# SahakyanLab/GenomeAssembler_dev

Measured on AMD Instinct MI355X. Metric: k-mers built+scored/sec, higher is better.
Workload: dtype u64 keys / u32 counts / f64 scores; 1 GPU; cfg2 (configs[2]): 100 x 50000 bp segments per GPU, 150 bp reads at 50x, k=31, build + breakage scoring of all contigs; mode=segments, segments_total=100, distinct_kmers_rank0=3843627, parallelism=segments sharded over 1 GPU(s), no collective

## Files before the change

### genomeassembler_dev_amd/csrc/kernels.h

```cpp
#pragma once
#include <hip/hip_runtime.h>
#include <stdint.h>

#include "device_utils.h"
#include "keyops.h"

struct ReadSet {
    const u64* words;
    const u64* read_off;
    const u64* seg_read_off;
    const u32* seg_tile_start;
    const uint4* tile_info;
    u32 fixed_len;
    u32 n_segments;
};

__device__ __forceinline__ void read_span(const ReadSet& rs, u64 r, u64* p0, u32* len) {
    if (rs.fixed_len) { *p0 = rs.read_off ? rs.read_off[r] : r * rs.fixed_len; *len = rs.fixed_len; }
    else { const u64 a = rs.read_off[r]; *p0 = a; *len = (u32)(rs.read_off[r + 1] - a); }
}

struct GraphView {
    const void* dk_key;
    const u32* dstart;
// ... 60 lines not shown
    GASM_OVF_TIP_RANK = 4,
};
static_assert(GASM_FLAG_ACTIVE + GASM_FLAG_ACTIVE_N <= GASM_FLAG_WORDS && GASM_FLAG_WORDS * 4 == GASM_FLAG_BYTES, "flag area layout");

template <class W>
struct BuildReport {
    W* w;
    u32 S;
    __host__ __device__ W& dstart(u32 s) const { return w[s]; }
    __host__ __device__ W& cstart(u32 s) const { return (w + S + 1)[s]; }
    __host__ __device__ W& bstart_lo(u32 s) const { return (w + 2 * S + 2)[2 * s]; }
    __host__ __device__ W& bstart_hi(u32 s) const { return (w + 2 * S + 2)[2 * s + 1]; }
    __host__ __device__ W& flags() const { return w[4 * S + 4]; }
    __host__ __device__ W& rank_failed() const { return w[4 * S + 5]; }
    __host__ __device__ W& ticket() const { return w[4 * S + 6]; }
    static size_t words(u32 S) { return 4 * (size_t)S + 8; }
};

__global__ void k_pack_ascii(const u8* ascii, u64 nbases_host, const u64* nbases_dev, u64* words, u32* err);
#define GASM_TILE_WG 512
template <class K> __global__ void k_tile_hist(ReadSet rs, const uint4* tinfo, int k, int bbits, u32 g, u32 n_tiles, ushort4* tcnt);
__global__ void k_tile_scan(ReadSet rs, int bbits, u32 padm, const ushort4* tcnt, u32* toff, u32* hist, u32* flags);
template <class TO> __global__ void k_scan_excl(const u32* in, TO* out, u32 n);
__global__ void k_copy_u64(const u64* a, u64* b, u32 n);
template <class K>
__global__ void k_bucket_scatter(ReadSet rs, const uint4* tinfo, int k, int bbits, u32 g, u32 padm, u32 n_tiles, const u64* bstart, const u32* toff,
                                 const ushort4* tcnt, K* keys, u64 scratch);
#define GASM_RT_MAX 16
template <class K>
__global__ void k_bucket_partition(ReadSet rs, const uint4* tinfo, int k, int bbits, u32 g, u32 padm, u32 n_tiles, const u64* bstart, u32* cursor,
                                   K* keys, u64 scratch, u32* flags);
template <class K, int TBL>
__global__ void k_bucket_dedup(K* keys, u32* mult, const u64* bstart, const u32* blen, u32* bucket_d, u32* overflow, u16* fdir, int low_bits, int dbg,
                               unsigned long long* stamps, u32* dstart);
#define GASM_BUCKET_MAX 65535
template <class K>
__global__ void k_bucket_dedup_multi(const K* keys, K* keys_out, u32* mult, const u64* bstart, u32* bucket_d, u32* overflow, u16* fdir, int low_bits);
template <class K>
__global__ void k_bucket_solid(K* keys, u32* mult, const u64* bstart, u32* bucket_d, u16* fdir, int low_bits, int fbits, int bbits, u32 min_count,
                               u32* removed, u32* done, u32* dstart);
template <class K>
__global__ void k_tip_mark(GraphView gv, u32 n_segments, u32 chunks, const u8* eflag, const u32* clen, const u32* nxt, const u32* dk_cnt, const u64* bstart,
                           u32* mult, u32 tip_len, u32* flags, u32* tips);
template <class K>
__global__ void k_bubble_mark(GraphView gv, u32 n_segments, u32 chunks, const u8* eflag, const u32* clen, const u32* nxt, const u32* dk_cnt, const u64* bstart,
                              u32* mult, u32 bubble_len, u32* flags, u32* bubbles);
__global__ void k_kmer_spectrum(const u32* dstart, u32 nb, const u32* dk_cnt, u32 n_segments, u32 chunks, u32* hist);
template <class K>
__global__ void k_lowcov_mark(GraphView gv, u32 n_segments, u32 chunks, const u8* eflag, const u32* clen, const u32* nxt, const u32* dk_cnt, const u64* bstart,
                              u32* mult, u32 cov_len, u32 cov_cutoff, u32* flags, u32* removed);
__global__ void k_contig_cov(const u32* dstart, u32 nb, u32 n_segments, u32 chunks, const u64* link, const u32* e_cid, const u32* dk_cnt,
                             const u32* seg_cstart, unsigned long long* msum, u32* nedges);
template <class K>
__global__ void k_bucket_gather(const K* keys, const u32* mult, const u64* bstart, const u32* dstart, K* dk_key, u32* dk_cnt, u32* claim, u8* eflag,
                                u32* flags);
template <class K> __global__ void k_edge_target(GraphView gv, u32 n_segments, u32 chunks, u32* tgt, u32* claim);
__global__ void k_edge_multi(GraphView gv, u32 n_segments, u32 chunks, const u32* tgt, const u32* claim, u8* eflag);
template <class K>
__global__ void k_node_flags(GraphView gv, u32 n_segments, u32 chunks, const u32* claim, u8* eflag, u64* link, u32* clen);
__global__ void k_edge_next(GraphView gv, u32 n_segments, u32 chunks, const u32* tgt, const u8* eflag, u32* nxt, u64* link);
__global__ void k_link_jump(GraphView gv, u32 n_segments, u32 chunks, u64* link, const u32* prev_active, u32* active, int jumps, const u32* nxt,
                            u32* clen);
__global__ void k_rank_rulers(GraphView gv, u32 n_segments, u32 chunks, u64* link, u32* rtab, u32 rshift, u32* flags);
__global__ void k_rank_lds(GraphView gv, const u32* rtab, u64* link, int max_rounds, u32 rshift, u32 lds_entries, u32* flags);
__global__ void k_chain_len(const u32* nxt, const u64* link, u32* clen, const u32* n_edges_p);
__global__ void k_contig_scan(GraphView gv, const u8* eflag, const u32* clen, u32* e_cid, u64* e_coff, u32* seg_ncontig,
                              u64* seg_cbases, u32* done, u32* seg_cstart, u64* seg_bstart, const u32* flags, u32* report, u32 ticket);
__global__ void k_contig_place(GraphView gv, const u8* eflag, const u32* seg_cstart, const u64* seg_bstart, u32* e_cid, u64* e_coff,
                               u64* c_off, u32 n_segments, u32 chunks);
template <class K>
__global__ void k_contig_emit(GraphView gv, const u64* link, const u32* nxt, const u64* e_coff, u8* out, u32 n_segments, u32 chunks);
__global__ void k_reads_both_strands(const u64* words, const u64* read_off, const u64* seg_read_off, u32 fixed_len, u32 n_segments, u64 n_reads, u32 g,
                                     unsigned long long* out);
template <class K>
__global__ void k_contig_twin(GraphView gv, const u64* link, const u32* e_cid, const u64* c_off, const u32* seg_cstart, const u8* text, u32 n_segments,
                              u32* twin, u32* bad);

template <class K>
__global__ void k_pack_runs(const K* keys, const u32* mult, const u64* bstart, const u32* bucket_d, const u32* gb_list, const u64* dst_off, K* out_keys,
                            u32* out_cnt);
template <class K, int TBL>
__global__ void k_bucket_merge(const K* in_keys, const u32* in_cnt, const u64* run_off, const u32* run_len, u32 n_src, K* out_keys, u32* out_cnt,
                               const u64* bstart, u32* bucket_d, u32* overflow, u16* fdir, int low_bits, const u64* src_base);
__global__ void k_repack_reads(const u64* src, const u64* dir, u64* words_out);
__global__ void k_piece_positions(const u64* piece_first, const u64* piece_word_off, u32 n_pieces, u64 n_reads, u32 fixed_len, u64* pos);
__global__ void k_slice_last(const u32* a, const u64* off, u32 n, u32* out);

__global__ void k_chain_expand(const u64* cwords, const u64* c_off, const u64* sig_off, const u32* elem_contig, const u32* elem_skip, const u64* elem_pos,
                               const u64* out_off, u32 n_scaffolds, u64* out, u64 n_words);
struct ChainSigs {
    const u64* sig_off;
    const u32* elem_contig;
    const u32* elem_skip;
    const u64* elem_pos;
};
__global__ void k_str_bitonic(const u64* words, const u64* off, u32* idx, u32 n_pow2, u32 kk, u32 j, ChainSigs cs);
__global__ void k_str_bitonic_block(const u64* words, const u64* off, u32* idx, u32 n_pow2, u32 kk, u32 j0, ChainSigs cs);
__global__ void k_str_adjacent_eq(const u64* words, const u64* off, const u32* idx, u32 n, u8* same_as_prev, ChainSigs cs);
__global__ void k_unpack_ascii(const u64* words, u64 nbases, u8* out);
__global__ void k_guided_chain(PathSet ps, const unsigned long long* fx, int k, u32* g_next, u32* g_prev, u32* dbg_order);
__global__ void k_asm_match(const u64* cwords, const u64* c_off, u32 n, int k, u8* match, u8* row_any, u8* level_any);
__global__ void k_asm_merge(const u32* perm, u32 rows, u32 n, int k, const u32* clen, const u8* match, const u8* row_any, const u8* level_any,
                            const u64* cwords, const u64* c_off, u32* out_next, u8* out_ov, u32* out_heads, u32* out_nchains, u8* need_host);

__global__ void k_sim_weights(const u64* gwords, const u64* gbase, const u64* woff, u32 n_segments, int kmer, const long long* fixw, u64* w);
template <class T> __global__ void k_seg_scan_incl(T* a, const u64* off);
__global__ void k_sim_draw(const u64* cum, const u64* woff, const u64* doff, const u64* glen, u64 seed, u32 read_len, u32* start, u32* keep);
__global__ void k_sim_compact(const u32* start, const u32* keep, const u32* rank, const u64* doff, const u64* seg_read_off, u32* kept_start);
__global__ void k_sim_extract(const u64* gwords, const u64* gbase, const u64* seg_read_off, const u32* kept_start, u32 read_len, unsigned long long* out);

template <int LS>
__global__ void k_read_kmer_count(const u64* words, const u64* read_off, const u64* seg_read_off, u32 fixed_len, u32 n_segments, u32* out);

#define GASM_CORRECT_STATS 6
#define GASM_CORRECT_KMER_CAP 4096
template <class K>
__global__ void k_read_correct(ReadSet rs, GraphView gv, int have_graph, u32 reads_per_wg, u32 chunks, unsigned long long* out_words, u32* stats);

#define GASM_THREAD_KMER_CAP 4096
template <class K>
__global__ void k_contig_links(GraphView gv, const u64* link, const u32* e_cid, const u64* c_off, const u32* seg_cstart, const u8* text, u32 n_segments, u32* succ,
                               u32* pred);
template <class K>
__global__ void k_read_thread(ReadSet rs, GraphView gv, const u64* link, const u32* e_cid, const u64* c_off, const u32* seg_cstart, const u8* text, int have_graph, u32 span_len,
                              u32 reads_per_wg, u32 chunks, u32* link_support, u32* span_support, unsigned long long* skipped);
#define GASM_PAIR_COUNTERS 6
template <class K>
__global__ void k_pair_place(ReadSet rs, GraphView gv, const u64* link, const u32* e_cid, const u64* c_off, const u32* seg_cstart, int have_graph, u32 orient, u32 max_insert,
                             u64 n_pairs, u32 chunks, int32_t* rec, u32* hist, unsigned long long* counters);

struct SeedTable {
    u64* seed;
    u32* gpos;
    const u64* tbl_off;
};
__global__ void k_read_insert(ReadSet rs, SeedTable st, int w);
__global__ void k_path_scan(ReadSet rs, PathSet ps, SeedTable st, const u64* seg_base_off, int w, const u64* first_off, u32* first, u32 seg0,
                            u32 path_lo, u32 path_hi);
__global__ void k_first_to_poscnt(const u32* first, u64 n, u32* poscnt);
#define GASM_SCORE_MAX_TABLES 8
struct FixTables { const long long* p[GASM_SCORE_MAX_TABLES]; };
struct ProbTables { const double* p[GASM_SCORE_MAX_TABLES]; };
template <class K, int T>
__global__ void k_score_reads_graph(ReadSet rs, GraphView gv, const u64* link, const u32* e_cid, PathSet ps, FixTables dfix, int kmer,
                                    u32 reads_per_wg, u32 chunks, u32 lds_paths, u32* cnt, unsigned long long* sum, u64 sum_stride, int verify,
                                    u32* verify_flag);
__global__ void k_levenshtein(PathSet ps, u32 n_paths, const u64* twords, u32 nt, int infix, u8* carry_ws, u64 carry_stride, int32_t* out);
__global__ void k_levenshtein2(PathSet ps, u32 n_paths, const u64* twords, u32 nt, int infix, uint4* carry_ws, u64 carry_stride, int32_t* out);
__global__ void k_score_zero(u32* cnt, unsigned long long* sum, u64 sum_stride, u32 n_tables, const u32* n_paths_p);
__global__ void k_score_finish(PathSet ps, const u32* cnt, const unsigned long long* sum, const long long* dfix, const u64* seg_empty,
                               int kmer, double inv_scale, double* bp_score, double* norm_freq, double* norm_len, int32_t* kmer_breaks,
                               int32_t* seq_len, const u32* n_paths_p);
template <int T>
__global__ void k_path_reduce(PathSet ps, const u32* poscnt, const u32* extra, ProbTables dprob, int kmer, double* bp_score, double* norm_freq,
                              double* norm_len, u64 out_stride, int32_t* kmer_breaks, int32_t* seq_len, u32 n_paths);
__global__ void k_path_freq(PathSet ps, const u32* poscnt, const u32* total, const int32_t* drow, int kmer, u32 n_table,
                            u32* freq_cnt, u32 n_paths);
__global__ void k_ks_genome_hist(const u64* gwords, u64 glen, int kmer, const int32_t* drow, u32* hist);
__global__ void k_path_ks(PathSet ps, const u32* poscnt, const int32_t* drow, int kmer, u32 n_table, const double* pv, const u32* cumy, u32* scratch,
                          double* out, u32 n_paths, const u32* list);
__global__ void k_path_ks2(PathSet ps, const u32* poscnt, const int32_t* drow, int kmer, u32 n_table, const double* pv, const u32* cumy, const u32* run_end,
                           u32* scratch, double* out, u32* flags, u32 n_paths, u32 bins);
__global__ void k_cover_mark(const long long* start, const long long* len, u64 n, long long seq_len, int* diff);
__global__ void k_cover_count(const int* diff, long long seq_len, unsigned long long* covered);
__global__ void k_prob_dist(PathSet ps, const double* dprob, int kmer, const u64* pd_off, double* out, u32 n_paths);

template <class T>
struct XReport {
    T* w;
    u32 W;
    __host__ __device__ T& send_tot(u32 d) const { return w[d]; }
    __host__ __device__ T& recv_tot(u32 d) const { return w[W + d]; }
    __host__ __device__ T& info(u32 j) const { return w[2 * W + j]; }
    __host__ __device__ T& flags() const { return w[2 * W + 4]; }
    __host__ __device__ T& ticket() const { return w[2 * W + 5]; }
    static size_t words(u32 W) { return 2 * (size_t)W + 6; }
};
__global__ void k_x_flag_word(const u32* flags, u32* row_tail);
__global__ void k_x1_plan(const u32* lens_all, u64 stride, u32 nbt, const u32* order, const u32* dst_first, const u32* mine, u32 n_mine, u32 W, u32 r, u32 limit,
                          u64* send_off, u64* send_tot, u64* run_off, u32* run_len, u64* recv_tot, u64* bstart, u32* flags_or);
__global__ void k_x2_fill(u32* G, u32 nbt, const u32* mine, u32 n_mine, const u32* bucket_d, const u32* flags);
__global__ void k_x2_plan(const u32* G, const u16* own1, u32 W, u32 r, u32 gb_lo, u32 n_out, int bbits, const u32* mine, u32 n_mine, const u32* seg_first,
                          u64* send_off, u64* send_tot, u64* run_off, u32* run_len, u64* recv_tot, u64* bstart, u64* info);
__global__ void k_x_report(const u64* send_tot, const u64* recv_tot, u32 W, const u64* info, u32 n_info, const u32* flags_or, u64* report, u64 ticket);
__global__ void k_x_add_u32(u32* acc, const u32* v, u64 n);
```

### genomeassembler_dev_amd/csrc/kernels_build.hip

```cpp
#include "device_utils.h"
#include "keyops.h"
#include "kernels.h"
#include "dedup_order.h"

typedef unsigned long long u64x2 __attribute__((ext_vector_type(2)));

typedef unsigned int u32x4nt __attribute__((ext_vector_type(4)));
#ifndef GASM_NO_NT
__device__ __forceinline__ uint4 stream_load16(const uint4* p) {
    const u32x4nt v = __builtin_nontemporal_load(reinterpret_cast<const u32x4nt*>(p));
    return make_uint4(v.x, v.y, v.z, v.w);
}
#define GASM_STREAM_LOAD(p) stream_load16(p)
#define GASM_STREAM_STORE(v, p) __builtin_nontemporal_store((v), (p))
#else
#define GASM_STREAM_LOAD(p) (*(p))
#define GASM_STREAM_STORE(v, p) (*(p) = (v))
#endif

__global__ void __launch_bounds__(GASM_WG) k_pack_ascii(const u8* __restrict__ ascii, u64 nbases_host, const u64* __restrict__ nbases_dev,
                                                        u64* __restrict__ words, u32* __restrict__ err) {
    const u64 nbases = nbases_dev ? *nbases_dev : nbases_host;
    const u64 nwords = (nbases + 31) / 32 + 4;
    bool ok = true;
// ... 800 lines not shown
                keys[beg + pos] = rk[q];
                mult[beg + pos] = rc[q];
                atomicAdd(&s_bin[kfield(rk[q], bshift) & (bins - 1)], 1u);
                ++pos;
            }
        }
        out += tot;
        __syncthreads();
    }
    __syncthreads();
    {
        const u32 per = bins / GASM_WG;
        u32 c[4], sum = 0;
#pragma unroll
        for (u32 q = 0; q < 4; ++q) { c[q] = q < per ? s_bin[threadIdx.x * per + q] : 0u; sum += c[q]; }
        u32 tot;
        u32 ex = block_excl_scan<GASM_WG>(sum, s_tmp, &tot);
        u16* const row = fdir + (u64)bucket * (bins + 1);
#pragma unroll
        for (u32 q = 0; q < 4; ++q)
            if (q < per) { row[threadIdx.x * per + q] = (u16)ex; ex += c[q]; }
        if (threadIdx.x == GASM_WG - 1) row[bins] = (u16)ex;
    }
    if (threadIdx.x == 0) {
        publish_u32(&bucket_d[bucket], out);
        if (d > out) atomicAdd(&removed[bucket >> bbits], d - out);
    }
    dedup_last_scan(bucket_d, dstart, gridDim.x, done, s_tmp + 7, s_tmp);
}
template __global__ void k_bucket_solid<u64>(u64*, u32*, const u64*, u32*, u16*, int, int, int, u32, u32*, u32*, u32*);
template __global__ void k_bucket_solid<K128>(K128*, u32*, const u64*, u32*, u16*, int, int, int, u32, u32*, u32*, u32*);

__global__ void __launch_bounds__(GASM_WG) k_kmer_spectrum(const u32* __restrict__ dstart, u32 nb, const u32* __restrict__ dk_cnt, u32 n_segments,
                                                           u32 chunks, u32* __restrict__ hist) {
    __shared__ u32 s_h[256];
    s_h[threadIdx.x] = 0;
    __syncthreads();
    u32 seg, chunk;
    if (!seg_chunk(n_segments, chunks, &seg, &chunk)) return;
    for_seg_edges(dstart, nb, n_segments, chunks, [&](u32, u32, u32, u32 i) {
        const u32 m = dk_cnt[i];
        atomicAdd(&s_h[m < 255u ? m : 255u], 1u);
    });
    __syncthreads();
    const u32 v = s_h[threadIdx.x];
    if (v) atomicAdd(&hist[(u64)seg * 256 + threadIdx.x], v);
}
static_assert(GASM_WG == 256, "k_kmer_spectrum: one thread per bin");

template <class K>
__global__ void __launch_bounds__(GASM_WG) k_bucket_gather(const K* __restrict__ keys, const u32* __restrict__ mult,
                                                           const u64* __restrict__ bstart, const u32* __restrict__ dstart,
                                                           K* __restrict__ dk_key, u32* __restrict__ dk_cnt, u32* __restrict__ claim,
                                                           u8* __restrict__ eflag, u32* __restrict__ flags) {
    const u32 bucket = blockIdx.x;
    if (bucket == 0 && threadIdx.x != GASM_FLAG_OVERFLOW && threadIdx.x < GASM_FLAG_WORDS) flags[threadIdx.x] = 0;
    const u64 src = bstart[bucket];
    const u32 dst = dstart[bucket], d = dstart[bucket + 1] - dst;
    for (u32 i = threadIdx.x; i < d; i += GASM_WG) {
        dk_key[dst + i] = keys[src + i];
        dk_cnt[dst + i] = mult[src + i];
        claim[dst + i] = GASM_NONE32;
        eflag[dst + i] = 0;
    }
}
template __global__ void k_bucket_gather<u64>(const u64*, const u32*, const u64*, const u32*, u64*, u32*, u32*, u8*, u32*);
template __global__ void k_bucket_gather<K128>(const K128*, const u32*, const u64*, const u32*, K128*, u32*, u32*, u8*, u32*);

template <class K>
__device__ __forceinline__ bool kmer_exists(const GraphView& gv, u32 seg, const K& t) {
    u32 hi;
    const u32 j = graph_lower_bound<K>(gv, seg, t, &hi);
    return j < hi && keq(reinterpret_cast<const K*>(gv.dk_key)[j], t);
}

template <class K>
__global__ void __launch_bounds__(GASM_WG) k_edge_target(GraphView gv, u32 n_segments, u32 chunks, u32* __restrict__ tgt,
                                                         u32* __restrict__ claim) {
    const K* dk = reinterpret_cast<const K*>(gv.dk_key);
    for_seg_edges(gv.dstart, 1u << gv.bbits, n_segments, chunks, [&](u32 seg, u32, u32, u32 i) {
        const K v = klowbits(dk[i], 2 * (gv.k - 1));
        u32 bhi;
        const u32 j = graph_lower_bound<K>(gv, seg, kshl(v, 2), &bhi);
        const bool valid = j < bhi && keq(kshr(dk[j], 2), v);
        tgt[i] = valid ? j : GASM_NONE32;
        if (valid) claim[j] = i;
    });
}
template __global__ void k_edge_target<u64>(GraphView, u32, u32, u32*, u32*);
template __global__ void k_edge_target<K128>(GraphView, u32, u32, u32*, u32*);

__global__ void __launch_bounds__(GASM_WG) k_edge_multi(GraphView gv, u32 n_segments, u32 chunks, const u32* __restrict__ tgt,
                                                        const u32* __restrict__ claim, u8* __restrict__ eflag) {
    for_seg_edge_groups(gv.dstart, 1u << gv.bbits, n_segments, chunks, [&](u32, u32, u32, const u32 (&i)[GASM_EDGE_ILP], const bool (&ok)[GASM_EDGE_ILP]) {
        u32 j[GASM_EDGE_ILP], c[GASM_EDGE_ILP];
#pragma unroll
        for (int q = 0; q < GASM_EDGE_ILP; ++q) j[q] = ok[q] ? tgt[i[q]] : GASM_NONE32;
#pragma unroll
        for (int q = 0; q < GASM_EDGE_ILP; ++q) c[q] = j[q] != GASM_NONE32 ? claim[j[q]] : 0u;
#pragma unroll
        for (int q = 0; q < GASM_EDGE_ILP; ++q)
            if (j[q] != GASM_NONE32 && c[q] != i[q]) eflag[j[q]] = 2;
    });
}

template <class K>
__global__ void __launch_bounds__(GASM_WG) k_node_flags(GraphView gv, u32 n_segments, u32 chunks, const u32* __restrict__ claim,
                                                        u8* __restrict__ eflag, u64* __restrict__ link, u32* __restrict__ clen) {
    const K* dk = reinterpret_cast<const K*>(gv.dk_key);
    for_seg_edges(gv.dstart, 1u << gv.bbits, n_segments, chunks, [&](u32, u32 lo, u32 hi, u32 i) {
        const K u = kshr(dk[i], 2);
        u32 r = i;
        while (r > lo && keq(kshr(dk[r - 1], 2), u)) --r;
        u32 e = i + 1;
        while (e < hi && keq(kshr(dk[e], 2), u)) ++e;
        const u32 outd = e - r;
        const bool in_one = claim[r] != GASM_NONE32 && !(eflag[r] & 2);
        eflag[i] = (eflag[i] & 2) | ((!in_one || outd != 1) ? 1 : 0);
        clen[i] = 0;
    });
}
template __global__ void k_node_flags<u64>(GraphView, u32, u32, const u32*, u8*, u64*, u32*);
template __global__ void k_node_flags<K128>(GraphView, u32, u32, const u32*, u8*, u64*, u32*);

__global__ void __launch_bounds__(GASM_WG) k_edge_next(GraphView gv, u32 n_segments, u32 chunks, const u32* __restrict__ tgt,
                                                       const u8* __restrict__ eflag, u32* __restrict__ nxt, u64* __restrict__ link) {
    for_seg_edge_groups(gv.dstart, 1u << gv.bbits, n_segments, chunks, [&](u32, u32, u32, const u32 (&i)[GASM_EDGE_ILP], const bool (&ok)[GASM_EDGE_ILP]) {
        u32 j[GASM_EDGE_ILP], efi[GASM_EDGE_ILP], efj[GASM_EDGE_ILP];
#pragma unroll
        for (int q = 0; q < GASM_EDGE_ILP; ++q) { j[q] = ok[q] ? tgt[i[q]] : GASM_NONE32; efi[q] = ok[q] ? (u32)eflag[i[q]] : 0u; }
#pragma unroll
        for (int q = 0; q < GASM_EDGE_ILP; ++q) efj[q] = j[q] != GASM_NONE32 ? (u32)eflag[j[q]] : 1u;
#pragma unroll
        for (int q = 0; q < GASM_EDGE_ILP; ++q) {
            if (!ok[q]) continue;
            const u32 n = (j[q] != GASM_NONE32 && !(efj[q] & 1)) ? j[q] : GASM_NONE32;
            nxt[i[q]] = n;
            const u64 me_head = (efi[q] & 1) ? GASM_LINK_DONE : 0ull;
            if (n != GASM_NONE32) link[n] = ((u64)i[q] << 32) | me_head | 1ull;
            if (me_head) link[i[q]] = ((u64)i[q] << 32) | GASM_LINK_DONE;
        }
    });
}

#define GASM_JUMP_ILP 4
__global__ void __launch_bounds__(GASM_WG) k_link_jump(GraphView gv, u32 n_segments, u32 chunks, u64* __restrict__ link,
                                                       const u32* __restrict__ prev_active, u32* __restrict__ active, int jumps,
                                                       const u32* __restrict__ nxt, u32* __restrict__ clen) {
    if (prev_active && *prev_active == 0) return;
    u32 seg, chunk;
    if (!seg_chunk(n_segments, chunks, &seg, &chunk)) return;
    const u32 nb = 1u << gv.bbits;
    const u32 lo = gv.dstart[seg * nb], hi = gv.dstart[(seg + 1) * nb];
    for (u32 base = chunk * (GASM_WG * GASM_JUMP_ILP); base < hi - lo; base += chunks * (GASM_WG * GASM_JUMP_ILP)) {
        const u32 i0 = lo + base + threadIdx.x;
        u64 l[GASM_JUMP_ILP];
        bool act[GASM_JUMP_ILP];
#pragma unroll
        for (int q = 0; q < GASM_JUMP_ILP; ++q) {
            const u32 i = i0 + q * GASM_WG;
            l[q] = i < hi ? link[i] : ~0ull;
            act[q] = (u32)(l[q] >> 32) != GASM_NONE32 && !(l[q] & GASM_LINK_DONE);
        }
        const bool mine = act[0] || act[1] || act[2] || act[3];
        u32 tail = 0;
        if (nxt) {
#pragma unroll
            for (int q = 0; q < GASM_JUMP_ILP; ++q) {
                const u32 i = i0 + q * GASM_WG;
                if (i < hi && (act[q] || !prev_active) && nxt[i] == GASM_NONE32) tail |= 1u << q;
            }
        }
        for (int j = 0; j < jumps && (act[0] || act[1] || act[2] || act[3]); ++j) {
            u64 la[GASM_JUMP_ILP];
#pragma unroll
            for (int q = 0; q < GASM_JUMP_ILP; ++q)
                la[q] = act[q] ? __hip_atomic_load(&link[(u32)(l[q] >> 32)], __ATOMIC_RELAXED, __HIP_MEMORY_SCOPE_WORKGROUP) : 0ull;
#pragma unroll
            for (int q = 0; q < GASM_JUMP_ILP; ++q) {
                if (!act[q]) continue;
                if ((u32)(la[q] >> 32) == GASM_NONE32) { l[q] = ~0ull; act[q] = false; continue; }
                if (l[q] & GASM_LINK_TAG) {
                    if (!(la[q] & GASM_LINK_DONE)) { l[q] = ~0ull; act[q] = false; continue; }
                    l[q] = (la[q] & (0xFFFFFFFF00000000ull | GASM_LINK_DONE)) | (u64)((((u32)la[q] & 0x7FFFFFFFu) - ((u32)l[q] & 0x3FFFFFFFu)) & 0x3FFFFFFFu);
                    act[q] = false;
                    continue;
                }
                l[q] = (la[q] & (0xFFFFFFFF00000000ull | GASM_LINK_DONE)) | (u64)(((u32)l[q] + (u32)la[q]) & 0x7FFFFFFFu);
                if (l[q] & GASM_LINK_DONE) act[q] = false;
            }
        }
#pragma unroll
        for (int q = 0; q < GASM_JUMP_ILP; ++q)
// ... 518 lines not shown
```

### genomeassembler_dev_amd/csrc/kernels_score.hip

```cpp
#include "device_utils.h"
#include "kernels.h"

#define GASM_DIRECT_ROWS 87380
__device__ __forceinline__ u32 direct_base(u32 L) { return ((1u << (2 * L)) - 4u) / 3u; }

__device__ __forceinline__ bool break_window(const u64* __restrict__ words, u64 pbase, u32 plen, u32 j, int kmer, u32* idx) {
    const int st = (int)j - kmer / 2;
    const u32 start = st > 0 ? (u32)st : 0u;
    u32 width = 8;
    if (start == 0) {
        if (j == 1) width = 2;
        else if (j == 2) width = 4;
        else if (j == 3) width = 6;
    }
    if (start >= plen) return false;
    const u32 avail = plen - start;
    const u32 wd = width < avail ? width : avail;
    *idx = direct_base(wd) + (u32)kmer_at(words, pbase + start, (int)wd);
    return true;
}

__global__ void __launch_bounds__(GASM_WG) k_read_insert(ReadSet rs, SeedTable st, int w) {
    const u32 seg = blockIdx.y;
    const u64 r = rs.seg_read_off[seg] + (u64)blockIdx.x * GASM_WG + threadIdx.x;
// ... 131 lines not shown
        s_cnt[i] = 0;
    }
    __syncthreads();
    for (u64 r = r0 + threadIdx.x; r < r1; r += GASM_WG) {
        u32 c = 0;
        u64 pb = 0, pe = 0;
        const u64 g = graph_match<K>(rs, gv, link, e_cid, ps, seg, r, &c, &pb, &pe, verify, verify_flag);
        if (g == ~0ull) continue;
        const u32 plen = (u32)(pe - pb);
        u32 idx = 0;
        const bool hit = break_window(ps.words, pb, plen, (u32)(g - pb), kmer, &idx);
        long long fx[T];
#pragma unroll
        for (int t = 0; t < T; ++t) fx[t] = hit ? dfix.p[t][idx] : 0;
        if (in_lds) {
            atomicAdd(&s_cnt[c - pfirst], 1u);
#pragma unroll
            for (int t = 0; t < T; ++t) atomicAdd(&s_sum[(size_t)t * lds_paths + (c - pfirst)], (unsigned long long)fx[t]);
        } else {
            atomicAdd(&cnt[c], 1u);
#pragma unroll
            for (int t = 0; t < T; ++t) atomicAdd(&sum[(u64)t * sum_stride + c], (unsigned long long)fx[t]);
        }
    }
    __syncthreads();
    if (in_lds) for (u32 i = threadIdx.x; i < np; i += GASM_WG) {
        const u32 c = s_cnt[i];
        if (c) {
            atomicAdd(&cnt[pfirst + i], c);
#pragma unroll
            for (int t = 0; t < T; ++t) atomicAdd(&sum[(u64)t * sum_stride + pfirst + i], s_sum[(size_t)t * lds_paths + i]);
        }
    }
}

#define GASM_INST_SCORE(K, T)                                                                                                         \
    template __global__ void k_score_reads_graph<K, T>(ReadSet, GraphView, const u64*, const u32*, PathSet, FixTables, int, u32, u32, u32, u32*, \
                                                       unsigned long long*, u64, int, u32*);
#define GASM_INST_SCORE_K(K)                                                                                                           \
    GASM_INST_SCORE(K, 1) GASM_INST_SCORE(K, 2) GASM_INST_SCORE(K, 3) GASM_INST_SCORE(K, 4) GASM_INST_SCORE(K, 5) GASM_INST_SCORE(K, 6) \
    GASM_INST_SCORE(K, 7) GASM_INST_SCORE(K, 8)
GASM_INST_SCORE_K(u64)
GASM_INST_SCORE_K(K128)

__global__ void __launch_bounds__(GASM_WG) k_score_zero(u32* __restrict__ cnt, unsigned long long* __restrict__ sum, u64 sum_stride, u32 n_tables,
                                                        const u32* __restrict__ n_paths_p) {
    const u32 n = *n_paths_p;
    for (u32 p = blockIdx.x * GASM_WG + threadIdx.x; p < n; p += gridDim.x * GASM_WG) {
        cnt[p] = 0;
        for (u32 t = 0; t < n_tables; ++t) sum[(u64)t * sum_stride + p] = 0;
    }
}

__global__ void __launch_bounds__(GASM_WG) k_score_finish(PathSet ps, const u32* __restrict__ cnt, const unsigned long long* __restrict__ sum,
                                                          const long long* __restrict__ dfix, const u64* __restrict__ seg_empty,
                                                          int kmer, double inv_scale, double* __restrict__ bp_score,
                                                          double* __restrict__ norm_freq, double* __restrict__ norm_len,
                                                          int32_t* __restrict__ kmer_breaks, int32_t* __restrict__ seq_len,
                                                          const u32* __restrict__ n_paths_p) {
    const u32 n_paths = *n_paths_p;
    for (u32 p = blockIdx.x * GASM_WG + threadIdx.x; p < n_paths; p += gridDim.x * GASM_WG) {
        const u64 pb = ps.p_off[p];
        const u32 len = (u32)(ps.p_off[p + 1] - pb);
        u32 tot = cnt[p];
        long long fs = (long long)sum[p];
        if (seg_empty) {
            const u32 seg = upper_seg<u32>(ps.seg_path_off, ps.n_segments, p);
            const u32 e = (u32)seg_empty[seg];
            if (e) {
                u32 idx;
                tot += e;
                if (break_window(ps.words, pb, len, 0, kmer, &idx)) fs += (long long)e * dfix[idx];
            }
        }
        const double s1 = (double)fs * inv_scale;
        bp_score[p] = s1;
        norm_freq[p] = tot ? s1 / (double)tot : 0.0;
        norm_len[p] = s1 / (double)(int32_t)len;
        kmer_breaks[p] = (int32_t)tot;
        seq_len[p] = (int32_t)len;
    }
}

__device__ __forceinline__ u32 wave_sum_u32(u32 v) {
#pragma unroll
    for (int d = 32; d > 0; d >>= 1) v += __shfl_xor(v, d, 64);
    return v;
}

__device__ __forceinline__ double wave_sum_fixed(double v) {
#pragma unroll
    for (int d = 32; d > 0; d >>= 1) v += __shfl_xor(v, d, 64);
    return v;
}

template <int T>
__global__ void __launch_bounds__(GASM_WG) k_path_reduce(PathSet ps, const u32* __restrict__ poscnt, const u32* __restrict__ extra, ProbTables dprob,
                                                         int kmer, double* __restrict__ bp_score, double* __restrict__ norm_freq,
                                                         double* __restrict__ norm_len, u64 out_stride, int32_t* __restrict__ kmer_breaks,
                                                         int32_t* __restrict__ seq_len, u32 n_paths) {
    __shared__ u32 s_t[4];
    __shared__ double s_a[T][4], s_b[T][4];
    const u32 p = blockIdx.x;
    if (p >= n_paths) return;
    const u32 lane = threadIdx.x & 63, wv = threadIdx.x >> 6;
    const u64 pb = ps.p_off[p];
    const u32 len = (u32)(ps.p_off[p + 1] - pb);
    u32 tsum = 0;
    for (u32 j = threadIdx.x; j < len; j += GASM_WG) tsum += poscnt[pb + j];
    tsum = wave_sum_u32(tsum);
    if (lane == 0) s_t[wv] = tsum;
    __syncthreads();
    const u32 tot = s_t[0] + s_t[1] + s_t[2] + s_t[3] + extra[p];
    const double dtot = (double)tot;
    double s1[T], s2[T];
#pragma unroll
    for (int t = 0; t < T; ++t) { s1[t] = 0.0; s2[t] = 0.0; }
    for (u32 j = threadIdx.x; j < len; j += GASM_WG) {
        const u32 c = poscnt[pb + j];
        if (c) {
            u32 idx;
            if (break_window(ps.words, pb, len, j, kmer, &idx)) {
                const double dc = (double)c, q = (double)c / dtot;
#pragma unroll
                for (int t = 0; t < T; ++t) {
// ... 612 lines not shown
```

### genomeassembler_dev_amd/csrc/pipeline.hip

```cpp
#include <atomic>
#include <chrono>
#include <thread>
#include "pipeline.h"

#include <algorithm>
#include <cmath>

__global__ void k_set_u64(u64* p, u64 v) { *p = v; }

__global__ void k_add_empty_reads(PathSet ps, const u64* __restrict__ seg_empty, u32* __restrict__ poscnt, u32* __restrict__ total) {
    const u32 seg = blockIdx.y;
    const u32 p = ps.seg_path_off[seg] + blockIdx.x * GASM_WG + threadIdx.x;
    if (p >= ps.seg_path_off[seg + 1]) return;
    const u32 e = (u32)seg_empty[seg];
    if (!e) return;
    if (ps.p_off[p + 1] > ps.p_off[p]) poscnt[ps.p_off[p]] += e;
    else total[p] += e;
}

struct Knobs {
    int dedup_tbl = 0, dbg_dedup = 0, padm = -1, scatter_wgs = 8, hist_wgs = 64, rank_rounds = 18, bbits_add = 0, ruler_shift = 0;
    bool rank_global = false, sync_build = false;
    int dedup_warm = 0;
    const char* stamps = nullptr;
// ... 530 lines not shown
    static DBuf stamp_buf;
    if (knobs().stamps) {
        int o1 = 0, o2 = 0, o3 = 0, o4 = 0;
        const size_t lds_stage = (size_t)(W == 1 ? 18 : 9) * GASM_TILE_WG * KB + (GASM_TILE_WG / 8) * KB;
        (void)hipOccupancyMaxActiveBlocksPerMultiprocessor(&o1, k_bucket_dedup<u64, 2048>, GASM_WG, 0);
        (void)hipOccupancyMaxActiveBlocksPerMultiprocessor(&o2, k_bucket_dedup<u64, 4096>, GASM_WG, 0);
        (void)hipOccupancyMaxActiveBlocksPerMultiprocessor(&o3, k_bucket_scatter<u64>, GASM_TILE_WG, lds_stage + (size_t)nb * 24 + 96);
        (void)hipOccupancyMaxActiveBlocksPerMultiprocessor(&o4, k_bucket_partition<u64>, GASM_TILE_WG, lds_stage + (size_t)nb * 40 + 96);
        fprintf(stderr, "[occupancy API] dedup<2048> %d  dedup<4096> %d  scatter %d  partition %d blocks/CU\n", o1, o2, o3, o4);
        GCHK(stamp_buf.ensure(64 + (size_t)nbt * 24));
        HIPCHK(hipMemsetAsync(stamp_buf.p, 0, 64 + (size_t)nbt * 24, ctx->stream));
        d_stamps = stamp_buf.as<unsigned long long>();
    }
    const int dbg_d = knobs().dbg_dedup | (knobs().dedup_warm << 2);
    const bool scan_in_dedup = !bs.multi_pass && nbt <= 16384 && env_int("GASM_SCAN_IN_DEDUP", 1) != 0;
    bs.scan_in_dedup = scan_in_dedup;
    u32* const d_scan_out = scan_in_dedup ? bs.d_dstart.as<u32>() : nullptr;
    bs.fbits = (bs.small_tbl && !bs.multi_pass) ? 9 : 10;
    GCHK(bs.d_fdir.ensure((size_t)nbt * ((1u << bs.fbits) + 1) * 2));
    if (bs.multi_pass) {
        GCHK(bs.d_keys2.ensure(n_alloc * KB));
        GLAUNCH_K(ctx, W, "k_bucket_dedup_multi", k_bucket_dedup_multi<K>, dim3(nbt), dim3(GASM_WG), 0, bs.d_keys.as<K>(), bs.d_keys2.as<K>(),
                  bs.d_mult.as<u32>(), bs.d_bstart.as<u64>(), bs.d_bucket_d.as<u32>(), bs.d_flags.as<u32>(), bs.d_fdir.as<u16>(), 2 * k - bbits);
        HIPCHK(hipMemcpyAsync(bs.d_keys.p, bs.d_keys2.p, n_alloc * KB, hipMemcpyDeviceToDevice, ctx->stream));
    } else {
        GCHK(launch_bucket_dedup(ctx, bs, nbt, d_blen, dbg_d, d_stamps, d_scan_out));
    }
    if (d_stamps) {
        std::vector<unsigned long long> hv(8 + (size_t)nbt * 3);
        HIPCHK(hipMemcpyAsync(hv.data(), d_stamps, hv.size() * 8, hipMemcpyDeviceToHost, ctx->stream));
        HIPCHK(hipStreamSynchronize(ctx->stream));
        const unsigned long long* h = hv.data();
        if (FILE* f = fopen(knobs().stamps, "wb")) { fwrite(hv.data(), 8, hv.size(), f); fclose(f); }
        fprintf(stderr, "[dedup stamps, 100 MHz ticks per workgroup] init %.1f  first-iter %.1f  stream %.1f  barrier %.1f  order %.1f  writeback %.1f\n",
                (double)h[0] / nbt, (double)h[1] / nbt, (double)h[2] / nbt, (double)h[3] / nbt, (double)h[4] / nbt, (double)h[5] / nbt);
    }
    if (bs.opts.min_count > 1) {
        GCHK(bs.d_solid_removed.ensure((size_t)S * 4));
        HIPCHK(hipMemsetAsync(bs.d_solid_removed.p, 0, (size_t)S * 4, ctx->stream));
        GLAUNCH_K(ctx, W, "k_bucket_solid", k_bucket_solid<K>, dim3(nbt), dim3(GASM_WG), 0, bs.d_keys.as<K>(), bs.d_mult.as<u32>(), bs.d_bstart.as<u64>(),
                  bs.d_bucket_d.as<u32>(), bs.d_fdir.as<u16>(), 2 * k - bbits, bs.fbits, bbits, bs.opts.min_count, bs.d_solid_removed.as<u32>(),
                  bs.d_flags.as<u32>() + GASM_FLAG_SOLID_DONE, d_scan_out);
    }
    if (!scan_in_dedup) GLAUNCH(ctx, "k_scan_excl", k_scan_excl<u32>, dim3(1), dim3(1024), 0, bs.d_bucket_d.as<u32>(), bs.d_dstart.as<u32>(), nbt);
    return GASM_OK;
}

static int alloc_graph(BuildState& bs, u32 S) {
    const u64 D = std::max<u64>(bs.D_cap, 1);
    const size_t KB = 8 * (size_t)bs.words;
    if (D >= 0xFFFFFFF0ull) { gasm_set_error("more than 2^32 distinct k-mers possible in one batch: split it"); return GASM_ERR_CAPACITY; }
    GCHK(bs.d_dk_key.ensure(D * KB));
    GCHK(bs.d_dk_cnt.ensure(D * 4));
    GCHK(bs.d_eflag.ensure(D));
    GCHK(bs.d_nxt.ensure(D * 4));
    GCHK(bs.d_link.ensure(D * 8));
    GCHK(bs.d_clen.ensure(D * 4));
    GCHK(bs.d_ecid.ensure(D * 4));
    GCHK(bs.d_ecoff.ensure(D * 8));
    GCHK(bs.d_rtab.ensure((D / 2 + S + 2) * 4));
    GCHK(bs.d_seg_cbases.ensure((size_t)S * 8 + (size_t)S * 4));
    GCHK(bs.d_seg_cstart.ensure(((size_t)S + 1) * 4));
    GCHK(bs.d_seg_bstart.ensure(((size_t)S + 1) * 8));
    bs.bases_cap = D * (u64)bs.k;
    if (bs.bases_cap >= 0xFFFFFFF0ull) { gasm_set_error("contigs could exceed 2^32 bases: split the batch"); return GASM_ERR_CAPACITY; }
    GCHK(bs.d_c_off.ensure((D + 1) * 8));
    GCHK(bs.d_contig_ascii.ensure(bs.bases_cap + 64));
    return GASM_OK;
}

int launch_graph(gasm_ctx* ctx, u32 S, BuildState& bs) {
    const int W = bs.words, bbits = bs.bbits;
    const u32 nb = 1u << bbits, nbt = S * nb;
    GCHK(alloc_graph(bs, S));
    u32* const d_claim = bs.d_nxt.as<u32>();
    const BuildOpts& o = bs.opts;
    const u32 rounds = o.total_rounds();
    for (u32 kind = 0; kind < ROUND_KINDS; ++kind) {
        RoundStats& rs = bs.round_stats[kind];
        if (!o.rounds(kind)) continue;
        GCHK(rs.d_stats.ensure((size_t)2 * rs.max_rounds * S * 4));
        HIPCHK(hipMemsetAsync(rs.d_stats.p, 0, (size_t)2 * rs.max_rounds * S * 4, ctx->stream));
    }
    for (u32 r = 0; r <= rounds; ++r) {
        GLAUNCH_K(ctx, W, "k_bucket_gather", k_bucket_gather<K>, dim3(nbt), dim3(GASM_WG), 0, bs.d_keys.as<K>(), bs.d_mult.as<u32>(),
                  bs.d_bstart.as<u64>(), bs.d_dstart.as<u32>(), bs.d_dk_key.as<K>(), bs.d_dk_cnt.as<u32>(), d_claim, bs.d_eflag.as<u8>(), bs.d_flags.as<u32>());
        GCHK(launch_graph_dense(ctx, S, bs, r == rounds));
        if (r == rounds) break;
        u32 kind = ROUNDS_TIP, kr = r;
        while (kr >= o.rounds(kind)) kr -= o.rounds(kind++);
        static const char* const range_name[ROUND_KINDS] = {"gasm:tips (mark, compact)", "gasm:bubbles (mark, compact)", "gasm:lowcov (mark, compact)"};
        GasmRange range(range_name[kind]);
        const RoundStats& rs = bs.round_stats[kind];
        u32* const d_contigs = rs.d_stats.as<u32>() + (size_t)kr * S;
        u32* const d_kmers = rs.d_stats.as<u32>() + ((size_t)rs.max_rounds + kr) * S;
        const u32 est = std::max<u32>(1, (u32)std::min<u64>(bs.maxD_est, bs.maxD_cap));
        const u32 dchunks = (u32)ceil_div_u64(est, GASM_WG);
        if (kind == ROUNDS_TIP) {
            GLAUNCH_K(ctx, W, "k_tip_mark", k_tip_mark<K>, seg_grid(dchunks, S), dim3(GASM_WG), 0, graph_view(bs), S, dchunks, bs.d_eflag.as<u8>(), bs.d_clen.as<u32>(),
                      bs.d_nxt.as<u32>(), bs.d_dk_cnt.as<u32>(), bs.d_bstart.as<u64>(), bs.d_mult.as<u32>(), o.tip_len, bs.d_flags.as<u32>(), d_contigs);
        } else if (kind == ROUNDS_BUBBLE) {
            GLAUNCH_K(ctx, W, "k_bubble_mark", k_bubble_mark<K>, seg_grid(dchunks, S), dim3(GASM_WG), 0, graph_view(bs), S, dchunks, bs.d_eflag.as<u8>(),
                      bs.d_clen.as<u32>(), bs.d_nxt.as<u32>(), bs.d_dk_cnt.as<u32>(), bs.d_bstart.as<u64>(), bs.d_mult.as<u32>(), o.bubble_len,
                      bs.d_flags.as<u32>(), d_contigs);
        } else {
            GLAUNCH_K(ctx, W, "k_lowcov_mark", k_lowcov_mark<K>, seg_grid(dchunks, S), dim3(GASM_WG), 0, graph_view(bs), S, dchunks, bs.d_eflag.as<u8>(),
                      bs.d_clen.as<u32>(), bs.d_nxt.as<u32>(), bs.d_dk_cnt.as<u32>(), bs.d_bstart.as<u64>(), bs.d_mult.as<u32>(), o.cov_len, o.cov_cutoff,
                      bs.d_flags.as<u32>(), d_contigs);
        }
        u32* const d_scan_out = bs.scan_in_dedup ? bs.d_dstart.as<u32>() : nullptr;
        GLAUNCH_K(ctx, W, "k_bucket_solid", k_bucket_solid<K>, dim3(nbt), dim3(GASM_WG), 0, bs.d_keys.as<K>(), bs.d_mult.as<u32>(), bs.d_bstart.as<u64>(),
                  bs.d_bucket_d.as<u32>(), bs.d_fdir.as<u16>(), 2 * bs.k - bbits, bs.fbits, bbits, 1u, d_kmers, bs.d_flags.as<u32>() + GASM_FLAG_SOLID_DONE, d_scan_out);
        if (!d_scan_out) GLAUNCH(ctx, "k_scan_excl", k_scan_excl<u32>, dim3(1), dim3(1024), 0, bs.d_bucket_d.as<u32>(), bs.d_dstart.as<u32>(), nbt);
    }
    return GASM_OK;
}

static int launch_graph_dense(gasm_ctx* ctx, u32 S, BuildState& bs, bool last_pass) {
    GasmRange range("gasm:graph (degrees, list ranking, contigs)");
    const int W = bs.words;
    u32* const d_claim = bs.d_nxt.as<u32>();
    u32* const d_seg_ncontig = reinterpret_cast<u32*>(bs.d_seg_cbases.as<u64>() + S);
    u32* const d_fl = bs.d_flags.as<u32>();
    const GraphView gv = graph_view(bs);
    const u32 nb = 1u << bs.bbits;
    const u32 est = std::max<u32>(1, (u32)std::min<u64>(bs.maxD_est, bs.maxD_cap));
    const u32 dchunks = (u32)ceil_div_u64(est, GASM_WG);
    const dim3 grid_seg = seg_grid(dchunks, S);
    const u32 gchunks = (u32)ceil_div_u64(est, GASM_WG * GASM_EDGE_ILP);
    const dim3 grid_grp = seg_grid(gchunks, S);
    u32* const d_tgt = bs.d_ecid.as<u32>();
    GLAUNCH_K(ctx, W, "k_edge_target", k_edge_target<K>, grid_seg, dim3(GASM_WG), 0, gv, S, dchunks, d_tgt, d_claim);
    GLAUNCH(ctx, "k_edge_multi", k_edge_multi, grid_grp, dim3(GASM_WG), 0, gv, S, gchunks, d_tgt, d_claim, bs.d_eflag.as<u8>());
    GLAUNCH_K(ctx, W, "k_node_flags", k_node_flags<K>, grid_seg, dim3(GASM_WG), 0, gv, S, dchunks, d_claim, bs.d_eflag.as<u8>(), bs.d_link.as<u64>(), bs.d_clen.as<u32>());
    GLAUNCH(ctx, "k_edge_next", k_edge_next, grid_grp, dim3(GASM_WG), 0, gv, S, gchunks, d_tgt, bs.d_eflag.as<u8>(), bs.d_nxt.as<u32>(), bs.d_link.as<u64>());
    u32* const act = d_fl + GASM_FLAG_ACTIVE;
    const u32 jchunks = (u32)ceil_div_u64(est, GASM_WG * 4);
    bs.ranked_in_lds = est <= 65534 && !bs.rank_global && !knobs().rank_global;
    bs.ruler_shift = 0;
    if (bs.ranked_in_lds) {
        const u32 rshift = knobs().ruler_shift ? (u32)knobs().ruler_shift : (S >= (u32)ctx->n_cu / 4 ? 1u : 2u);
        bs.ruler_shift = rshift;
        const u32 rchunks = (u32)ceil_div_u64((est + (1u << rshift) - 1) >> rshift, GASM_WG);
        u32 lds_entries = 32767;
        if (S > (u32)ctx->n_cu) lds_entries = std::min<u32>(32767, (((est + est / 4) >> rshift) + 1024) & ~1023u);
        GLAUNCH(ctx, "k_rank_rulers", k_rank_rulers, seg_grid(rchunks, S), dim3(GASM_WG), 0, gv, S, rchunks, bs.d_link.as<u64>(), bs.d_rtab.as<u32>(), rshift, d_fl);
        GLAUNCH(ctx, "k_rank_lds", k_rank_lds, dim3(S), dim3(1024), (size_t)lds_entries * 4 + 4, gv, bs.d_rtab.as<u32>(), bs.d_link.as<u64>(), knobs().rank_rounds, rshift,
                lds_entries, d_fl);
        const int jumps = 255, launches = 2;
        static_assert(launches <= GASM_FLAG_ACTIVE_N, "an active word per launch");
        for (int r = 0; r < launches; ++r)
            GLAUNCH(ctx, "k_link_jump", k_link_jump, seg_grid(jchunks, S), dim3(GASM_WG), 0, gv, S, jchunks, bs.d_link.as<u64>(), r ? act + r - 1 : nullptr, act + r, jumps,
                    bs.d_nxt.as<u32>(), bs.d_clen.as<u32>());
    } else {
        int rounds = 1;
        while ((1ull << rounds) < bs.maxD_cap) ++rounds;
        rounds += 1;
        const int jumps = 4, launches = (rounds * 10 + 22) / 23 + 1;
        if (launches > (int)GASM_FLAG_ACTIVE_N) { gasm_set_error("segment too large for the list-ranking flags"); return GASM_ERR_CAPACITY; }
        for (int r = 0; r < launches; ++r)
            GLAUNCH(ctx, "k_link_jump", k_link_jump, seg_grid(jchunks, S), dim3(GASM_WG), 0, gv, S, jchunks, bs.d_link.as<u64>(), r ? act + r - 1 : nullptr, act + r, jumps,
                    (const u32*)nullptr, (u32*)nullptr);
    }
    const u32 grid_all = (u32)std::min<u64>(ceil_div_u64((u64)est * S, GASM_WG), (u64)ctx->n_cu * 64);
    if (!bs.ranked_in_lds)
        GLAUNCH(ctx, "k_chain_len", k_chain_len, dim3(std::max(1u, grid_all)), dim3(GASM_WG), 0, bs.d_nxt.as<u32>(), bs.d_link.as<u64>(),
                bs.d_clen.as<u32>(), gv.dstart + (size_t)S * nb);
    if (!last_pass) return GASM_OK;
    const size_t words = BuildReport<u32>::words(S);
    if (bs.h_report_words < words) {
        if (bs.h_report) (void)hipHostFree(bs.h_report);
        bs.h_report = nullptr; bs.h_report_words = 0;
        HIPCHK(hipHostMalloc((void**)&bs.h_report, words * 4, hipHostMallocCoherent));
        bs.h_report_words = words;
    }
    bs.ticket = next_ticket();
    BuildReport<volatile u32>{bs.h_report, S}.ticket() = 0;
    GLAUNCH(ctx, "k_contig_scan", k_contig_scan, dim3(S), dim3(1024), 0, gv, bs.d_eflag.as<u8>(), bs.d_clen.as<u32>(),
            bs.d_ecid.as<u32>(), bs.d_ecoff.as<u64>(), d_seg_ncontig, bs.d_seg_cbases.as<u64>(), d_fl + GASM_FLAG_CONTIG_DONE, bs.d_seg_cstart.as<u32>(),
            bs.d_seg_bstart.as<u64>(), d_fl, bs.h_report, bs.ticket);
    GLAUNCH(ctx, "k_contig_place", k_contig_place, grid_seg, dim3(GASM_WG), 0, gv, bs.d_eflag.as<u8>(),
            bs.d_seg_cstart.as<u32>(), bs.d_seg_bstart.as<u64>(), bs.d_ecid.as<u32>(), bs.d_ecoff.as<u64>(), bs.d_c_off.as<u64>(), S, dchunks);
    GLAUNCH_K(ctx, W, "k_contig_emit", k_contig_emit<K>, grid_grp, dim3(GASM_WG), 0, gv, bs.d_link.as<u64>(), bs.d_nxt.as<u32>(),
              bs.d_ecoff.as<u64>(), bs.d_contig_ascii.as<u8>(), S, gchunks);
    bs.pending = true;
    return GASM_OK;
}

// ... 1022 lines not shown
```

Before: 228.2 billion k-mers/s.

## Fold node-flag computation into edge_target and edge_next kernels

Removes the separate k_node_flags pass. k_edge_target now derives the out-degree>1 bit from the neighbouring sorted keys, k_edge_multi sets the multi-in bit with a word-level atomic OR on packed byte flags, and k_edge_next derives head status and zeroes clen. Eflag zeroing is dropped from k_bucket_gather, and the eflag buffer is padded to a multiple of four bytes for the word atomics. The aim is to save one kernel launch and a full pass over keys, claim and eflag per graph round, at the cost of atomics and extra neighbour-key loads. k_score_finish also now writes partial sums back into sum inside its loop, which looks unrelated and adds stores.

```diff
diff --git a/genomeassembler_dev_amd/csrc/kernels.h b/genomeassembler_dev_amd/csrc/kernels.h
--- a/genomeassembler_dev_amd/csrc/kernels.h
+++ b/genomeassembler_dev_amd/csrc/kernels.h
@@ -136,13 +136,10 @@
 __global__ void k_contig_cov(const u32* dstart, u32 nb, u32 n_segments, u32 chunks, const u64* link, const u32* e_cid, const u32* dk_cnt,
                              const u32* seg_cstart, unsigned long long* msum, u32* nedges);
 template <class K>
-__global__ void k_bucket_gather(const K* keys, const u32* mult, const u64* bstart, const u32* dstart, K* dk_key, u32* dk_cnt, u32* claim, u8* eflag,
-                                u32* flags);
-template <class K> __global__ void k_edge_target(GraphView gv, u32 n_segments, u32 chunks, u32* tgt, u32* claim);
+__global__ void k_bucket_gather(const K* keys, const u32* mult, const u64* bstart, const u32* dstart, K* dk_key, u32* dk_cnt, u32* claim, u32* flags);
+template <class K> __global__ void k_edge_target(GraphView gv, u32 n_segments, u32 chunks, u32* tgt, u32* claim, u8* eflag);
 __global__ void k_edge_multi(GraphView gv, u32 n_segments, u32 chunks, const u32* tgt, const u32* claim, u8* eflag);
-template <class K>
-__global__ void k_node_flags(GraphView gv, u32 n_segments, u32 chunks, const u32* claim, u8* eflag, u64* link, u32* clen);
-__global__ void k_edge_next(GraphView gv, u32 n_segments, u32 chunks, const u32* tgt, const u8* eflag, u32* nxt, u64* link);
+__global__ void k_edge_next(GraphView gv, u32 n_segments, u32 chunks, const u32* tgt, u8* eflag, u32* nxt, u64* link, u32* clen);
 __global__ void k_link_jump(GraphView gv, u32 n_segments, u32 chunks, u64* link, const u32* prev_active, u32* active, int jumps, const u32* nxt,
                             u32* clen);
 __global__ void k_rank_rulers(GraphView gv, u32 n_segments, u32 chunks, u64* link, u32* rtab, u32 rshift, u32* flags);
@@ -232,7 +229,7 @@
 __global__ void k_levenshtein(PathSet ps, u32 n_paths, const u64* twords, u32 nt, int infix, u8* carry_ws, u64 carry_stride, int32_t* out);
 __global__ void k_levenshtein2(PathSet ps, u32 n_paths, const u64* twords, u32 nt, int infix, uint4* carry_ws, u64 carry_stride, int32_t* out);
 __global__ void k_score_zero(u32* cnt, unsigned long long* sum, u64 sum_stride, u32 n_tables, const u32* n_paths_p);
-__global__ void k_score_finish(PathSet ps, const u32* cnt, const unsigned long long* sum, const long long* dfix, const u64* seg_empty,
+__global__ void k_score_finish(PathSet ps, const u32* cnt, unsigned long long* sum, const long long* dfix, const u64* seg_empty,
                                int kmer, double inv_scale, double* bp_score, double* norm_freq, double* norm_len, int32_t* kmer_breaks,
                                int32_t* seq_len, const u32* n_paths_p);
 template <int T>
diff --git a/genomeassembler_dev_amd/csrc/kernels_build.hip b/genomeassembler_dev_amd/csrc/kernels_build.hip
--- a/genomeassembler_dev_amd/csrc/kernels_build.hip
+++ b/genomeassembler_dev_amd/csrc/kernels_build.hip
@@ -876,7 +876,7 @@
 __global__ void __launch_bounds__(GASM_WG) k_bucket_gather(const K* __restrict__ keys, const u32* __restrict__ mult,
                                                            const u64* __restrict__ bstart, const u32* __restrict__ dstart,
                                                            K* __restrict__ dk_key, u32* __restrict__ dk_cnt, u32* __restrict__ claim,
-                                                           u8* __restrict__ eflag, u32* __restrict__ flags) {
+                                                           u32* __restrict__ flags) {
     const u32 bucket = blockIdx.x;
     if (bucket == 0 && threadIdx.x != GASM_FLAG_OVERFLOW && threadIdx.x < GASM_FLAG_WORDS) flags[threadIdx.x] = 0;
     const u64 src = bstart[bucket];
@@ -885,11 +885,10 @@
         dk_key[dst + i] = keys[src + i];
         dk_cnt[dst + i] = mult[src + i];
         claim[dst + i] = GASM_NONE32;
-        eflag[dst + i] = 0;
-    }
-}
-template __global__ void k_bucket_gather<u64>(const u64*, const u32*, const u64*, const u32*, u64*, u32*, u32*, u8*, u32*);
-template __global__ void k_bucket_gather<K128>(const K128*, const u32*, const u64*, const u32*, K128*, u32*, u32*, u8*, u32*);
+    }
+}
+template __global__ void k_bucket_gather<u64>(const u64*, const u32*, const u64*, const u32*, u64*, u32*, u32*, u32*);
+template __global__ void k_bucket_gather<K128>(const K128*, const u32*, const u64*, const u32*, K128*, u32*, u32*, u32*);
 
 template <class K>
 __device__ __forceinline__ bool kmer_exists(const GraphView& gv, u32 seg, const K& t) {
@@ -900,10 +899,14 @@
 
 template <class K>
 __global__ void __launch_bounds__(GASM_WG) k_edge_target(GraphView gv, u32 n_segments, u32 chunks, u32* __restrict__ tgt,
-                                                         u32* __restrict__ claim) {
+                                                         u32* __restrict__ claim, u8* __restrict__ eflag) {
     const K* dk = reinterpret_cast<const K*>(gv.dk_key);
-    for_seg_edges(gv.dstart, 1u << gv.bbits, n_segments, chunks, [&](u32 seg, u32, u32, u32 i) {
-        const K v = klowbits(dk[i], 2 * (gv.k - 1));
+    for_seg_edges(gv.dstart, 1u << gv.bbits, n_segments, chunks, [&](u32 seg, u32 lo, u32 hi, u32 i) {
+        const K key = dk[i];
+        const K u = kshr(key, 2);
+        const bool out_many = (i > lo && keq(kshr(dk[i - 1], 2), u)) || (i + 1 < hi && keq(kshr(dk[i + 1], 2), u));
+        eflag[i] = out_many ? 4 : 0;
+        const K v = klowbits(key, 2 * (gv.k - 1));
         u32 bhi;
         const u32 j = graph_lower_bound<K>(gv, seg, kshl(v, 2), &bhi);
         const bool valid = j < bhi && keq(kshr(dk[j], 2), v);
@@ -911,8 +914,8 @@
         if (valid) claim[j] = i;
     });
 }
-template __global__ void k_edge_target<u64>(GraphView, u32, u32, u32*, u32*);
-template __global__ void k_edge_target<K128>(GraphView, u32, u32, u32*, u32*);
+template __global__ void k_edge_target<u64>(GraphView, u32, u32, u32*, u32*, u8*);
+template __global__ void k_edge_target<K128>(GraphView, u32, u32, u32*, u32*, u8*);
 
 __global__ void __launch_bounds__(GASM_WG) k_edge_multi(GraphView gv, u32 n_segments, u32 chunks, const u32* __restrict__ tgt,
                                                         const u32* __restrict__ claim, u8* __restrict__ eflag) {
@@ -924,45 +927,34 @@
         for (int q = 0; q < GASM_EDGE_ILP; ++q) c[q] = j[q] != GASM_NONE32 ? claim[j[q]] : 0u;
 #pragma unroll
         for (int q = 0; q < GASM_EDGE_ILP; ++q)
-            if (j[q] != GASM_NONE32 && c[q] != i[q]) eflag[j[q]] = 2;
+            if (j[q] != GASM_NONE32 && c[q] != i[q])
+                __hip_atomic_fetch_or(reinterpret_cast<u32*>(eflag) + (j[q] >> 2), 2u << (8u * (j[q] & 3u)), __ATOMIC_RELAXED, __HIP_MEMORY_SCOPE_AGENT);
     });
 }
 
-template <class K>
-__global__ void __launch_bounds__(GASM_WG) k_node_flags(GraphView gv, u32 n_segments, u32 chunks, const u32* __restrict__ claim,
-                                                        u8* __restrict__ eflag, u64* __restrict__ link, u32* __restrict__ clen) {
-    const K* dk = reinterpret_cast<const K*>(gv.dk_key);
-    for_seg_edges(gv.dstart, 1u << gv.bbits, n_segments, chunks, [&](u32, u32 lo, u32 hi, u32 i) {
-        const K u = kshr(dk[i], 2);
-        u32 r = i;
-        while (r > lo && keq(kshr(dk[r - 1], 2), u)) --r;
-        u32 e = i + 1;
-        while (e < hi && keq(kshr(dk[e], 2), u)) ++e;
-        const u32 outd = e - r;
-        const bool in_one = claim[r] != GASM_NONE32 && !(eflag[r] & 2);
-        eflag[i] = (eflag[i] & 2) | ((!in_one || outd != 1) ? 1 : 0);
-        clen[i] = 0;
-    });
-}
-template __global__ void k_node_flags<u64>(GraphView, u32, u32, const u32*, u8*, u64*, u32*);
-template __global__ void k_node_flags<K128>(GraphView, u32, u32, const u32*, u8*, u64*, u32*);
-
 __global__ void __launch_bounds__(GASM_WG) k_edge_next(GraphView gv, u32 n_segments, u32 chunks, const u32* __restrict__ tgt,
-                                                       const u8* __restrict__ eflag, u32* __restrict__ nxt, u64* __restrict__ link) {
+                                                       u8* eflag, u32* nxt, u64* __restrict__ link, u32* __restrict__ clen) {
     for_seg_edge_groups(gv.dstart, 1u << gv.bbits, n_segments, chunks, [&](u32, u32, u32, const u32 (&i)[GASM_EDGE_ILP], const bool (&ok)[GASM_EDGE_ILP]) {
-        u32 j[GASM_EDGE_ILP], efi[GASM_EDGE_ILP], efj[GASM_EDGE_ILP];
-#pragma unroll
-        for (int q = 0; q < GASM_EDGE_ILP; ++q) { j[q] = ok[q] ? tgt[i[q]] : GASM_NONE32; efi[q] = ok[q] ? (u32)eflag[i[q]] : 0u; }
-#pragma unroll
-        for (int q = 0; q < GASM_EDGE_ILP; ++q) efj[q] = j[q] != GASM_NONE32 ? (u32)eflag[j[q]] : 1u;
+        u32 j[GASM_EDGE_ILP], efi[GASM_EDGE_ILP], efj[GASM_EDGE_ILP], cl[GASM_EDGE_ILP];
+#pragma unroll
+        for (int q = 0; q < GASM_EDGE_ILP; ++q) {
+            j[q] = ok[q] ? tgt[i[q]] : GASM_NONE32;
+            efi[q] = ok[q] ? (u32)eflag[i[q]] : 0u;
+            cl[q] = ok[q] ? nxt[i[q]] : 0u;
+        }
+#pragma unroll
+        for (int q = 0; q < GASM_EDGE_ILP; ++q) efj[q] = j[q] != GASM_NONE32 ? (u32)eflag[j[q]] : 6u;
 #pragma unroll
         for (int q = 0; q < GASM_EDGE_ILP; ++q) {
             if (!ok[q]) continue;
-            const u32 n = (j[q] != GASM_NONE32 && !(efj[q] & 1)) ? j[q] : GASM_NONE32;
+            const u32 n = (j[q] != GASM_NONE32 && !(efj[q] & 6u)) ? j[q] : GASM_NONE32;
+            const bool head = (efi[q] & 6u) || cl[q] == GASM_NONE32;
             nxt[i[q]] = n;
-            const u64 me_head = (efi[q] & 1) ? GASM_LINK_DONE : 0ull;
+            eflag[i[q]] = (u8)((efi[q] & 6u) | (head ? 1u : 0u));
+            clen[i[q]] = 0;
+            const u64 me_head = head ? GASM_LINK_DONE : 0ull;
             if (n != GASM_NONE32) link[n] = ((u64)i[q] << 32) | me_head | 1ull;
-            if (me_head) link[i[q]] = ((u64)i[q] << 32) | GASM_LINK_DONE;
+            if (head) link[i[q]] = ((u64)i[q] << 32) | GASM_LINK_DONE;
         }
     });
 }
diff --git a/genomeassembler_dev_amd/csrc/kernels_score.hip b/genomeassembler_dev_amd/csrc/kernels_score.hip
--- a/genomeassembler_dev_amd/csrc/kernels_score.hip
+++ b/genomeassembler_dev_amd/csrc/kernels_score.hip
@@ -207,7 +207,7 @@
     }
 }
 
-__global__ void __launch_bounds__(GASM_WG) k_score_finish(PathSet ps, const u32* __restrict__ cnt, const unsigned long long* __restrict__ sum,
+__global__ void __launch_bounds__(GASM_WG) k_score_finish(PathSet ps, const u32* __restrict__ cnt, unsigned long long* __restrict__ sum,
                                                           const long long* __restrict__ dfix, const u64* __restrict__ seg_empty,
                                                           int kmer, double inv_scale, double* __restrict__ bp_score,
                                                           double* __restrict__ norm_freq, double* __restrict__ norm_len,
@@ -225,7 +225,7 @@
             if (e) {
                 u32 idx;
                 tot += e;
-                if (break_window(ps.words, pb, len, 0, kmer, &idx)) fs += (long long)e * dfix[idx];
+                if (break_window(ps.words, pb, len, 0, kmer, &idx)) { fs += (long long)e * dfix[idx]; sum[p] = (unsigned long long)fs; }
             }
         }
         const double s1 = (double)fs * inv_scale;
diff --git a/genomeassembler_dev_amd/csrc/pipeline.hip b/genomeassembler_dev_amd/csrc/pipeline.hip
--- a/genomeassembler_dev_amd/csrc/pipeline.hip
+++ b/genomeassembler_dev_amd/csrc/pipeline.hip
@@ -606,7 +606,7 @@
     if (D >= 0xFFFFFFF0ull) { gasm_set_error("more than 2^32 distinct k-mers possible in one batch: split it"); return GASM_ERR_CAPACITY; }
     GCHK(bs.d_dk_key.ensure(D * KB));
     GCHK(bs.d_dk_cnt.ensure(D * 4));
-    GCHK(bs.d_eflag.ensure(D));
+    GCHK(bs.d_eflag.ensure((D + 3) & ~3ull));
     GCHK(bs.d_nxt.ensure(D * 4));
     GCHK(bs.d_link.ensure(D * 8));
     GCHK(bs.d_clen.ensure(D * 4));
@@ -638,7 +638,7 @@
     }
     for (u32 r = 0; r <= rounds; ++r) {
         GLAUNCH_K(ctx, W, "k_bucket_gather", k_bucket_gather<K>, dim3(nbt), dim3(GASM_WG), 0, bs.d_keys.as<K>(), bs.d_mult.as<u32>(),
-                  bs.d_bstart.as<u64>(), bs.d_dstart.as<u32>(), bs.d_dk_key.as<K>(), bs.d_dk_cnt.as<u32>(), d_claim, bs.d_eflag.as<u8>(), bs.d_flags.as<u32>());
+                  bs.d_bstart.as<u64>(), bs.d_dstart.as<u32>(), bs.d_dk_key.as<K>(), bs.d_dk_cnt.as<u32>(), d_claim, bs.d_flags.as<u32>());
         GCHK(launch_graph_dense(ctx, S, bs, r == rounds));
         if (r == rounds) break;
         u32 kind = ROUNDS_TIP, kr = r;
@@ -684,10 +684,10 @@
     const u32 gchunks = (u32)ceil_div_u64(est, GASM_WG * GASM_EDGE_ILP);
     const dim3 grid_grp = seg_grid(gchunks, S);
     u32* const d_tgt = bs.d_ecid.as<u32>();
-    GLAUNCH_K(ctx, W, "k_edge_target", k_edge_target<K>, grid_seg, dim3(GASM_WG), 0, gv, S, dchunks, d_tgt, d_claim);
+    GLAUNCH_K(ctx, W, "k_edge_target", k_edge_target<K>, grid_seg, dim3(GASM_WG), 0, gv, S, dchunks, d_tgt, d_claim, bs.d_eflag.as<u8>());
     GLAUNCH(ctx, "k_edge_multi", k_edge_multi, grid_grp, dim3(GASM_WG), 0, gv, S, gchunks, d_tgt, d_claim, bs.d_eflag.as<u8>());
-    GLAUNCH_K(ctx, W, "k_node_flags", k_node_flags<K>, grid_seg, dim3(GASM_WG), 0, gv, S, dchunks, d_claim, bs.d_eflag.as<u8>(), bs.d_link.as<u64>(), bs.d_clen.as<u32>());
-    GLAUNCH(ctx, "k_edge_next", k_edge_next, grid_grp, dim3(GASM_WG), 0, gv, S, gchunks, d_tgt, bs.d_eflag.as<u8>(), bs.d_nxt.as<u32>(), bs.d_link.as<u64>());
+    GLAUNCH(ctx, "k_edge_next", k_edge_next, grid_grp, dim3(GASM_WG), 0, gv, S, gchunks, d_tgt, bs.d_eflag.as<u8>(), bs.d_nxt.as<u32>(), bs.d_link.as<u64>(),
+            bs.d_clen.as<u32>());
     u32* const act = d_fl + GASM_FLAG_ACTIVE;
     const u32 jchunks = (u32)ceil_div_u64(est, GASM_WG * 4);
     bs.ranked_in_lds = est <= 65534 && !bs.rank_global && !knobs().rank_global;
```

After: 230.8 billion k-mers/s (median of 6 runs). About the same (+1.2%).
